# WangXuan95/NBLIC-Image-Compression

Measured on AMD Instinct MI355X. Metric: Mpixel/s encode (bit-exact) 4096x4096 gray -e1 lossless, higher is better.
Workload: dtype u8

## Files before the change

nblic-image-compression_amd/csrc/kernels_e1.h:

```cpp
#pragma once
#include <hip/hip_runtime.h>
#include <stdint.h>

namespace nblic {

constexpr uint32_t kMaxSegments = 1024;
constexpr uint32_t kTouchSegments = 256;
constexpr int kTotalsStride = 8, kWideTouchFlag = 4;
constexpr int kLongS2Met = 5, kLongS2Table = 6, kLongS2Serial = 7;
constexpr int kTotalsSlot = 16, kLongS3Split = 8, kLongS3Accepted = 9, kLongS3Missed = 10;
constexpr int kLongBlockMin = 128;

struct SegPlan { int nseg; uint32_t seg_len; };
SegPlan make_plan(uint32_t n_items, uint32_t max_segments = kMaxSegments);

constexpr size_t kStreamPad = 512;

struct E1Buffers {
    const uint8_t *img;
    uint32_t *rec1;
    uint16_t *s2in;
    uint32_t *pos2;
    uint16_t *s2out;
    uint16_t *pxs;
    uint16_t *s3in;
    uint32_t *pos3;
    uint16_t *s3out;
    uint8_t  *z;
    uint8_t  *cnt;
    uint32_t *ev_off;
    uint32_t *table;
    uint32_t *scan_sums;
    uint32_t *totals;
    int      *ctx_state;
    int      *map_state;
    int      *cnt_state;
    uint32_t *events;
    uint16_t *tin;
    uint64_t *tpos;
    uint16_t *tout;
    uint32_t *blk_base;
    int      *blk_end;
    uint8_t  *blk_ok;
    int      *blk_cand;
    uint32_t *blk_item;
    int      *blk_tab;
    uint32_t *mblk_base;
    uint32_t *mblk_cnt;
    uint32_t *mend_cnt;
    uint64_t *mblk_perm;
    uint32_t *qhist;
    unsigned long long *dbg_out;
    uint32_t *win_base;
    uint32_t *win_recs;
    uint16_t *coded;
};

struct E1Job {
    E1Buffers b;
    int h, w;
    uint32_t n;
    SegPlan pp;
    uint32_t n_ev;
    SegPlan pe;
    int dbg;
    int near, k_step;
    uint64_t ktab;
    int long_min, long_block;
    int row0;
    uint64_t *pack_rows;
    int pack_lane;
};

constexpr int kE1Kernels = 31;
constexpr int kE1Marks = kE1Kernels + 1;
struct E1Timers { hipEvent_t ev[kE1Marks]; uint64_t mask = ~0ull; };
constexpr uint64_t kRooflineStages = (1ull << 1) | (1ull << 26);
static const char *const kE1StageNames[kE1Kernels] = {
    "k_init_state", "k_predict",
    "k_adr_count", "scan_reduce.adr", "scan_sums.adr", "scan_apply.adr", "k_adr_scatter",
    "k_plan_blocks", "k_bias_blocks", "k_bias_fixup",
    "k_map_count", "scan_reduce.map", "scan_sums.map", "scan_apply.map", "k_map_scatter",
    "k_mapper_chains",
// ... 24 lines not shown
```

nblic-image-compression_amd/csrc/kernels_e1.hip:

```cpp
#include <hip/hip_runtime.h>
#include "model.h"
#include "kernels_e1.h"
#include "lsq_f64.h"
#include "serial_engine.h"

namespace nblic {

#define NB_GLOBAL __attribute__((address_space(1)))
typedef uint32_t u32x2 __attribute__((ext_vector_type(2)));
typedef uint32_t u32x4 __attribute__((ext_vector_type(4)));
typedef int i32x2 __attribute__((ext_vector_type(2)));
template <class T>
__device__ __forceinline__ NB_GLOBAL T *gptr(T *p) {
    return (NB_GLOBAL T *)p;
}

__device__ __forceinline__ int lane_id() { return int(threadIdx.x & 63); }
__device__ __forceinline__ uint64_t lanes_below() { return (1ull << lane_id()) - 1ull; }

__device__ __forceinline__ uint32_t xcd_block() {
    const uint32_t b = blockIdx.x, per = gridDim.x >> 3;
    return (b & 7u) * per + (b >> 3);
}

// ... 783 lines not shown
__global__ void __launch_bounds__(64) k_map_check(const E1Job *__restrict__ jobs) {
    __shared__ int count[kMapSyms][64];
    const E1Job &J = jobs[blockIdx.y];
    const auto base = gptr(J.b.mblk_base); const auto s3in = gptr(J.b.s3in); const auto s3out = gptr(J.b.s3out);
    const auto perm = gptr(J.b.mblk_perm); const auto cnt = gptr(J.b.mblk_cnt);
    const int lane = int(threadIdx.x);
    const int key = int(blockIdx.x) * kMapLanes + (lane < kMapLanes ? lane : 0);
    const uint32_t first = base[key], nb = lane < kMapLanes ? base[key + 1] - first : 0u;
    if (nb == 0u) return;
    uint32_t c_start, c_end;
    map_chain_range(J, key, c_start, c_end);
    const uint32_t B = map_block_records(J);
    Perm20 rank_of{perm[size_t(first) * 4 + 2], perm[size_t(first) * 4 + 3]};
    uint32_t accepted = 0, missed = 0;
    for (uint32_t b = 1; b < nb; b++) {
        const size_t it = size_t(first + b);
        if (perm[it * 4] == rank_of.lo && perm[it * 4 + 1] == rank_of.hi) {
            accepted++;
            rank_of = Perm20{perm[it * 4 + 2], perm[it * 4 + 3]};
            continue;
        }
        missed++;
        Perm20 sym_at{0, 0};
        for (int s = 0; s < kMapSyms; s++) {
            const int r = perm_get(rank_of, s);
            perm_set(sym_at, r, s); count[r][lane] = int(cnt[it * kMapSyms + s]);
        }
        const uint32_t lo = c_start + b * B, hi = min(c_end, lo + B);
        for (uint32_t r = lo; r < hi; r += 8u) {
            uint32_t y[8];
#pragma unroll
            for (int k = 0; k < 8; k++) y[k] = s3in[min(r + uint32_t(k), hi - 1u)];
#pragma unroll
            for (int k = 0; k < 8; k++)
                if (r + uint32_t(k) < hi) s3out[r + uint32_t(k)] = uint16_t(mapper_step(rank_of, sym_at, count, lane, int(y[k])));
        }
    }
    const auto st = gptr(J.b.map_state) + size_t(key) * (3 * kMapSyms);
    for (int s = 0; s < kMapSyms; s++) {
        const int r = perm_get(rank_of, s);
        st[s] = r; st[kMapSyms + r] = s; st[2 * kMapSyms + r] = int(gptr(J.b.mend_cnt)[key * kMapSyms + s]);
    }
    if (accepted) atomicAdd(J.b.totals + kLongS3Accepted, accepted);
    if (missed) atomicAdd(J.b.totals + kLongS3Missed, missed);
}

template <bool GEN, class Step>
__device__ __forceinline__ int walk_job(const E1Job &J, int qu, int qv, int z, Step step) {
    return GEN ? walk_symbol_t(J.k_step, J.ktab, qu, qv, z, step) : walk_symbol(kMinKStep, qu, qv, z, step);
}

template <bool GEN>
__global__ void __launch_bounds__(256) k_count_bins(const E1Job *__restrict__ jobs) {
    const E1Job &J = jobs[blockIdx.y];
    const auto rec1 = gptr(J.b.rec1); const auto s3out = gptr(J.b.s3out);
    const auto pos3 = gptr(J.b.pos3); const auto z = gptr(J.b.z); const auto cnt = gptr(J.b.cnt);
    uint32_t t = xcd_block() * 256u + threadIdx.x;
    if (t >= J.n) return;
    Level L = s1_level(rec1[t]);
    uint32_t p = pos3[t];
    int zz = (p >> 31) ? int(p & 0xFF) : int(s3out[p]);
    z[t] = uint8_t(zz);
    int c = 0;
    walk_job<GEN>(J, L.qu, L.qv, zz, [&](int, int, int, int bin) { c++; return bin; });
    cnt[t] = uint8_t(c);
}

template <bool GEN>
__global__ void __launch_bounds__(256) k_emit_bins(const E1Job *__restrict__ jobs) {
    const E1Job &J = jobs[blockIdx.y];
    const auto rec1 = gptr(J.b.rec1); const auto z = gptr(J.b.z);
    const auto ev_off = gptr(J.b.ev_off); const auto events = gptr(J.b.events);
    uint32_t t = xcd_block() * 256u + threadIdx.x;
    if (t >= J.n) return;
    Level L = s1_level(rec1[t]);
    auto out = events + ev_off[t];
    walk_job<GEN>(J, L.qu, L.qv, int(z[t]), [&](int qu, int qv, int node, int bin) {
        *out++ = pack_event(qu, qv, node, L.qw, bin);
        return bin;
    });
}

struct Touch { bool valid; uint32_t key; uint32_t payload; int slot; };

__device__ __forceinline__ Touch touch_of(uint32_t e, int parity) {
    const int qu = ev_qu(e), qv = ev_qv(e), node = ev_node(e), qw = ev_qw(e), bin = ev_bin(e);
    const bool same = qu == qv;
    const bool mine = (qu & 1) == parity;
    Touch t;
    t.valid = mine || (!same && qw != 0);
    const int tree = mine ? qu : qv;
    const int w1 = mine ? kWeightOne - qw : qw;
    t.slot = mine ? 0 : 1;
    t.key = uint32_t(parity) * 2048u + uint32_t(tree >> 1) * 256u + uint32_t(node);
    t.payload = uint32_t(w1) | (same ? uint32_t(qw) << 6 | 1u << 13 : 0u) | (uint32_t(bin) << 12);
    return t;
}

__global__ void __launch_bounds__(256) k_touch_count(const E1Job *__restrict__ jobs) {
    __shared__ uint32_t lds[4][4096];
    const E1Job &J = jobs[blockIdx.y];
    const auto events = gptr(J.b.events); const auto table = gptr(J.b.table);
    const uint32_t n_ev = J.n_ev; const SegPlan plan = J.pe;
    int seg = int(xcd_block()) * 4 + int(threadIdx.x >> 6);
    if (seg >= plan.nseg) return;
    if (seg == 0 && lane_id() == 0) gptr(J.b.totals)[kWideTouchFlag] = (J.dbg & 256) ? 1u : 0u;
    uint32_t *hist = lds[threadIdx.x >> 6];
    lds_fill<4096>(hist, 0);
    uint32_t lo = uint32_t(seg) * plan.seg_len, hi = min(n_ev, lo + plan.seg_len);
    for (uint32_t base = lo; base < hi; base += 512) {
        uint32_t e[8];
#pragma unroll
        for (int k = 0; k < 8; k++) e[k] = events[min(base + 64u * uint32_t(k) + uint32_t(lane_id()), hi - 1)];
#pragma unroll
        for (int k = 0; k < 8; k++) {
            if (base + 64u * uint32_t(k) + uint32_t(lane_id()) < hi) {
                Touch a = touch_of(e[k], 0), b = touch_of(e[k], 1);
                if (a.valid) atomicAdd(&hist[a.key], 1u);
                if (b.valid) atomicAdd(&hist[b.key], 1u);
            }
        }
    }
    for (int k = lane_id(); k < 4096; k += 64) table[size_t(k) * plan.nseg + seg] = hist[k];
}

constexpr int kStageSlots = 64, kStageRing = 64;
constexpr uint32_t kNoTouch = 0xFFFFFFFFu;
constexpr int kPosBits = 28;
constexpr uint32_t kPosMask = (1u << kPosBits) - 1u;
// ... 277 lines not shown
            vb_1 = c1 - (o_ex + (hw & one));
            const int slot = 2 + (n_halv < kMaxHalv ? n_halv : kMaxHalv);
            write_lane3(slot, H * kTpl + hk + 1, vb_s, vb_1, r0, r1, r2);
            n_halv++;
        }
        r2 = write_lane<1>(n_halv, r2);
        if (lane < 8) {
            const auto rec = recs + size_t(rec_i) * 24 + lane * 3;
            rec[0] = uint32_t(r0); rec[1] = uint32_t(r1); rec[2] = uint32_t(r2);
        }
        const uint32_t whole = read_lane(incl, 63);
        base_s = vb_s + int(whole >> 16);
        base_1 = vb_1 + int(whole & 0xFFFFu);
        n_halv_all += unsigned(n_halv);
        rec_i++;
    };
    const uint32_t last_window = first_window + ((end - 1 - first_window) / kWin) * kWin;
    auto fetch = [&](uint32_t window) { return in_w[(min(window, last_window) >> 3) + lane]; };
    u32x4 b0 = fetch(first_window), b1 = fetch(first_window + kWin), b2 = fetch(first_window + 2 * kWin), b3 = fetch(first_window + 3 * kWin);
    for (uint32_t window = first_window; window < end; window += 4 * kWin) {
        process(b0, window);
        b0 = fetch(window + 4 * kWin);
        if (window + kWin < end) process(b1, window + kWin);
        b1 = fetch(window + 5 * kWin);
        if (window + 2 * kWin < end) process(b2, window + 2 * kWin);
        b2 = fetch(window + 6 * kWin);
        if (window + 3 * kWin < end) process(b3, window + 3 * kWin);
        b3 = fetch(window + 7 * kWin);
    }
    if (lane == 0) cnt_state[key] = i32x2{base_s - base_1, base_1};
    if ((dbg & 8) && lane == 0 && end - start > 100000u) {
        const auto d = gptr(J.b.dbg_out) + 256 + (key & 255) * 4;
        d[0] = __builtin_amdgcn_s_memtime() - t_begin; d[1] = end - start; d[2] = rec_i - gptr(J.b.win_base)[key]; d[3] = n_halv_all;
    }
}

__global__ void __launch_bounds__(256) k_counter_probs(const E1Job *__restrict__ jobs) {
    const E1Job &J = jobs[blockIdx.y];
    const uint32_t g = blockIdx.x * 4u + (threadIdx.x >> 6);
    if (g >= gptr(J.b.win_base)[4096]) return;
    const int lane = lane_id();
    const auto r = (NB_GLOBAL const u32x4 *)gptr(J.b.win_recs) + size_t(g) * 6;
    const u32x4 r0 = r[0], r1 = r[1], r2 = r[2], r3 = r[3], r4 = r[4], r5 = r[5];
    const uint32_t window = r0.x, start = r0.y, end = r0.z;
    const int n_halv = min(int(r1.y), kMaxHalv + 1);
    const int from[kMaxHalv + 1] = {int(r1.z), int(r2.y), int(r3.x), int(r3.w), int(r4.z), int(r5.y)};
    const int hs[kMaxHalv + 1] = {int(r1.w), int(r2.z), int(r3.y), int(r4.x), int(r4.w), int(r5.z)};
    const int h1[kMaxHalv + 1] = {int(r2.x), int(r2.w), int(r3.z), int(r4.y), int(r5.x), int(r5.w)};
    const auto tin_g = gptr(J.b.tin); const auto tout = gptr(J.b.tout);
    const uint32_t first = window + uint32_t(lane) * kTpl;
    const u32x4 w = ((NB_GLOBAL const u32x4 *)tin_g)[first >> 3];
    uint32_t pay[kTpl]; int tin[kTpl], oin[kTpl], lane_t, lane_o;
    window_prefix(w, window, start, end, lane, pay, tin, oin, lane_t, lane_o);
    uint32_t p[kTpl];
#pragma unroll
    for (int k = 0; k < kTpl; k++) {
        const int j = lane * kTpl + k;
        int vs = int(r0.w), v1 = int(r1.x);
#pragma unroll
        for (int h = 0; h <= kMaxHalv; h++) if (h < n_halv && j >= from[h]) { vs = hs[h]; v1 = h1[h]; }
        const int t_ex = k ? tin[k - 1] : lane_t, o_ex = k ? oin[k - 1] : lane_o;
        p[k] = prob_one(v1 + o_ex, vs + t_ex);
    }
    if (first >= start && first + kTpl <= end) {
        ((NB_GLOBAL u32x4 *)tout)[first >> 3] = u32x4{p[0] | (p[1] << 16), p[2] | (p[3] << 16), p[4] | (p[5] << 16), p[6] | (p[7] << 16)};
    } else {
#pragma unroll
        for (int k = 0; k < kTpl; k++) if (first + k >= start && first + k < end) tout[first + k] = uint16_t(p[k]);
    }
}

__device__ __forceinline__ uint32_t mixed_code(const E1Job &J, uint32_t r, bool wide) {
    if (r >= J.n_ev) return 0u;
    const auto tout = gptr(J.b.tout);
    const auto pos0 = (NB_GLOBAL const uint32_t *)gptr(J.b.tpos);
    const auto pos1 = pos0 + ((size_t(J.n_ev) + 63) & ~size_t(63));
    uint32_t p0 = pos0[r], p1 = pos1[r];
    int qw, bin; bool odd;
    if (wide) {
        const uint32_t e = gptr(J.b.events)[r];
        qw = ev_qw(e); bin = ev_bin(e); odd = (ev_qu(e) & 1) != 0;
    } else {
        qw = int((p0 >> kPosBits) | (((p1 >> kPosBits) & 3u) << 4)); bin = int((p1 >> (kPosBits + 2)) & 1u); odd = (p1 >> 31) != 0u;
        p0 &= kPosMask; p1 &= kPosMask;
        if (p0 == kPosMask) p0 = kNoTouch;
        if (p1 == kPosMask) p1 = kNoTouch;
    }
    const uint32_t at_u = odd ? p1 : p0, other = odd ? p0 : p1, at_v = other == kNoTouch ? at_u : other;
    const int pu = tout[at_u], pv = tout[at_v];
    return uint32_t(mix_prob(pu, pv, qw)) | (uint32_t(bin) << 12);
}

__global__ void __launch_bounds__(256) k_mix(const E1Job *__restrict__ jobs) {
    const E1Job &J = jobs[blockIdx.y];
    const uint32_t r = xcd_block() * 256u + threadIdx.x;
    if ((r & ~63u) >= J.n_ev) return;
    const uint32_t code = mixed_code(J, r, gptr(J.b.totals)[kWideTouchFlag] != 0u);
    if (!J.pack_rows) {
        if (r < J.n_ev) gptr(J.b.coded)[r] = pack_coded(int(code & 0xFFFu), int(code >> 12));
        return;
    }
    const int lane = int(threadIdx.x) & 63;
    const int j = lane < kPackWords ? lane : kPackWords - 1;
    const uint32_t c0 = uint32_t(__builtin_amdgcn_ds_bpermute((4 * j + 0) << 2, int(code)));
    const uint32_t c1 = uint32_t(__builtin_amdgcn_ds_bpermute((4 * j + 1) << 2, int(code)));
    const uint32_t c2 = uint32_t(__builtin_amdgcn_ds_bpermute((4 * j + 2) << 2, int(code)));
    const uint32_t c3 = uint32_t(__builtin_amdgcn_ds_bpermute((4 * j + 3) << 2, int(code)));
    const uint32_t top_prob = uint32_t(__builtin_amdgcn_ds_bpermute((52 + (j < 12 ? j : 0)) << 2, int(code))) & 0xFFFu;
    const uint64_t ones = __ballot((code >> 12) != 0u);
    const uint64_t top = j < 12 ? uint64_t(top_prob) : ((ones >> 52) & 0xFFFull);
    const uint64_t word = uint64_t(c0) | (uint64_t(c1) << 13) | (uint64_t(c2) << 26) | (uint64_t(c3) << 39) | (top << 52);
    if (lane < kPackWords) ((NB_GLOBAL uint64_t *)gptr(J.b.tin))[size_t(r >> 6) * kPackWords + size_t(lane)] = word;
}

__global__ void __launch_bounds__(256) k_pack_rows(const E1Job *__restrict__ jobs, int n_jobs) {
// ... 17 lines not shown
    constexpr int kTile = 64;
    __shared__ int tile[kTile * 60];
    const IndexRecordTask T = tasks[blockIdx.x];
    const E1Job &J = jobs[T.job];
    const int t = int(threadIdx.x);
    const auto rec = gptr(out) + T.out;
    const auto words = (NB_GLOBAL uint32_t *)rec;
    constexpr int kHeadWords = int(sizeof(SerialState) / 4), kBiasWord = int(offsetof(SerialState, bias) / 4);
    if (t < kHeadWords) words[t] = t == kBiasWord ? uint32_t(lsq::kBiasInit) : 0u;
    const auto tab = words + kHeadWords;
    const auto ctx_state = gptr(J.b.ctx_state);
    for (int k = t; k < kContexts; k += 256) tab[k] = uint32_t(ctx_state[k]);
    const auto cnt_state = (NB_GLOBAL const i32x2 *)gptr(J.b.cnt_state);
    for (int key = t; key < 4096; key += 256) {
        const i32x2 c = cnt_state[key];
        const int tree = ((key >> 8) & 7) * 2 + (key >> 11), node = key & 255;
        tab[kContexts + tree * kTreeNodes + node] = uint32_t(c.x) | (uint32_t(c.y) << 16);
    }
    const auto map_state = gptr(J.b.map_state);
    const auto rank = rec + sizeof(SerialState) + size_t(kRecRank) * 4, sym = rec + sizeof(SerialState) + size_t(kRecSym) * 4;
    for (int m0 = 0; m0 < 512; m0 += kTile) {
        for (int k = t; k < kTile * 60; k += 256) tile[k] = map_state[m0 * 60 + k];
        __syncthreads();
        for (int k = t; k < kTile * kMapSyms; k += 256) {
            const int m = k / kMapSyms, q = k - m * kMapSyms;
            rank[m0 * kMapSyms + k] = uint8_t(tile[m * 60 + q]);
            sym[m0 * kMapSyms + k] = uint8_t(tile[m * 60 + 20 + q]);
            tab[kRecCount + m0 * kMapSyms + k] = uint32_t(tile[m * 60 + 40 + q]);
        }
        __syncthreads();
    }
    const int w = J.w, r = J.row0 + J.h, n = r < 2 ? r : 2;
    const auto rows = rec + kDecodeStateBytes;
    const auto img = gptr(J.b.img);
    const ptrdiff_t zeros = ptrdiff_t(2 - n) * w, from = ptrdiff_t(J.h - n) * w;
    for (ptrdiff_t k = t; k < 2 * ptrdiff_t(w); k += 256) rows[k] = k < zeros ? uint8_t(0) : img[from + (k - zeros)];
}

__global__ void k_init_state(const E1Job *__restrict__ jobs) {
    const E1Job &J = jobs[blockIdx.y];
    const auto ctx_state = gptr(J.b.ctx_state); const auto map_state = gptr(J.b.map_state); const auto cnt_state = (NB_GLOBAL i32x2 *)gptr(J.b.cnt_state);
    int g = int(blockIdx.x) * 256 + int(threadIdx.x);
    if (g < 3072) { ctx_state[g] = 0; gptr(J.b.qhist)[g] = 0; }
    if (g < 4096) cnt_state[g] = i32x2{kWeightOne, kWeightOne};
    if (g < 512)
        for (int k = 0; k < kMapSyms; k++) {
            map_state[g * 60 + k] = k; map_state[g * 60 + 20 + k] = k; map_state[g * 60 + 40 + k] = 2 * (kMapSyms - 1 - k);
        }
}

constexpr int kScanThreads = 256, kScanPerThread = 16, kScanTile = kScanThreads * kScanPerThread;

template <int WHICH> struct ScanSel;
template <> struct ScanSel<0> { typedef uint32_t T; static __device__ auto in(const E1Job &J) { return gptr(J.b.table); }  static __device__ auto out(const E1Job &J) { return gptr(J.b.table); }  static __device__ uint32_t n(const E1Job &J) { return uint32_t(kContexts) * J.pp.nseg; } };
template <> struct ScanSel<1> { typedef uint32_t T; static __device__ auto in(const E1Job &J) { return gptr(J.b.table); }  static __device__ auto out(const E1Job &J) { return gptr(J.b.table); }  static __device__ uint32_t n(const E1Job &J) { return 512u * J.pp.nseg; } };
template <> struct ScanSel<2> { typedef uint8_t  T; static __device__ auto in(const E1Job &J) { return gptr(J.b.cnt); }    static __device__ auto out(const E1Job &J) { return gptr(J.b.ev_off); } static __device__ uint32_t n(const E1Job &J) { return J.n; } };
template <> struct ScanSel<4> { typedef uint32_t T; static __device__ auto in(const E1Job &J) { return gptr(J.b.table); }  static __device__ auto out(const E1Job &J) { return gptr(J.b.table); }  static __device__ uint32_t n(const E1Job &J) { return 3072u * J.pp.nseg; } };
template <> struct ScanSel<3> { typedef uint32_t T; static __device__ auto in(const E1Job &J) { return gptr(J.b.table); }  static __device__ auto out(const E1Job &J) { return gptr(J.b.table); }  static __device__ uint32_t n(const E1Job &J) { return 4096u * J.pe.nseg; } };

template <int WHICH>
__global__ void __launch_bounds__(kScanThreads) k_scan_reduce(const E1Job *__restrict__ jobs) {
    __shared__ uint32_t part[kScanThreads / 64];
    const E1Job &J = jobs[blockIdx.y];
    const auto in = ScanSel<WHICH>::in(J);
    const uint32_t n = ScanSel<WHICH>::n(J);
    uint32_t base = blockIdx.x * uint32_t(kScanTile) + threadIdx.x * kScanPerThread, s = 0;
    if (blockIdx.x * uint32_t(kScanTile) >= n) return;
    for (int k = 0; k < kScanPerThread; k++) if (base + k < n) s += uint32_t(in[base + k]);
    s = wave_scan_incl(s);
    if (lane_id() == 63) part[threadIdx.x >> 6] = s;
    __syncthreads();
    if (threadIdx.x == 0) gptr(J.b.scan_sums)[blockIdx.x] = part[0] + part[1] + part[2] + part[3];
}

template <int WHICH>
__global__ void __launch_bounds__(1024) k_scan_sums(const E1Job *__restrict__ jobs) {
    __shared__ uint32_t part[16];
    __shared__ uint32_t carry;
    const E1Job &J = jobs[blockIdx.y];
    const auto sums = gptr(J.b.scan_sums);
    const uint32_t nblocks = (ScanSel<WHICH>::n(J) + kScanTile - 1) / kScanTile;
    if (threadIdx.x == 0) carry = 0;
    __syncthreads();
    for (uint32_t base = 0; base < nblocks; base += 1024) {
        uint32_t i = base + threadIdx.x;
        uint32_t v = i < nblocks ? sums[i] : 0u;
        uint32_t incl = wave_scan_incl(v);
        if (lane_id() == 63) part[threadIdx.x >> 6] = incl;
        __syncthreads();
        uint32_t pre = carry;
        for (int wv = 0; wv < int(threadIdx.x >> 6); wv++) pre += part[wv];
        if (i < nblocks) sums[i] = pre + incl - v;
        __syncthreads();
        if (threadIdx.x == 1023) carry = pre + incl;
        __syncthreads();
    }
    if (threadIdx.x == 0) {
        gptr(J.b.totals)[WHICH & 3] = carry;
        if (WHICH == 3 && carry >= kPosMask) gptr(J.b.totals)[kWideTouchFlag] = 1u;
    }
}

template <int WHICH>
__global__ void __launch_bounds__(kScanThreads) k_scan_apply(const E1Job *__restrict__ jobs) {
    __shared__ uint32_t part[kScanThreads / 64];
    const E1Job &J = jobs[blockIdx.y];
    const auto in = ScanSel<WHICH>::in(J);
    const auto out = ScanSel<WHICH>::out(J);
    const uint32_t n = ScanSel<WHICH>::n(J);
    if (blockIdx.x * uint32_t(kScanTile) >= n) return;
    uint32_t base = blockIdx.x * uint32_t(kScanTile) + threadIdx.x * kScanPerThread;
    uint32_t v[kScanPerThread], s = 0;
    for (int k = 0; k < kScanPerThread; k++) { v[k] = base + k < n ? uint32_t(in[base + k]) : 0u; s += v[k]; }
    uint32_t incl = wave_scan_incl(s);
    if (lane_id() == 63) part[threadIdx.x >> 6] = incl;
    __syncthreads();
    uint32_t pre = gptr(J.b.scan_sums)[blockIdx.x] + incl - s;
    for (int wv = 0; wv < int(threadIdx.x >> 6); wv++) pre += part[wv];
    for (int k = 0; k < kScanPerThread; k++) { if (base + k < n) out[base + k] = pre; pre += v[k]; }
}

__global__ void __launch_bounds__(256) k_q_predict(const E1Job *__restrict__ jobs) {
    const E1Job &J = jobs[blockIdx.z];
    const int w = J.w;
    int j = int(blockIdx.x) * 256 + int(threadIdx.x);
    int i = int(blockIdx.y);
    if (i >= J.h || j >= w) return;
    const auto img = gptr(J.b.img);
    auto pix = [&](int r, int c) { return int(img[size_t(r) * size_t(w) + size_t(c)]); };
    Taps n = sample_taps_q(pix, w, i, j);
    int px0 = predict_q(n);
    int err_prev = 0;
    if (j > 0) err_prev = pix(i, j - 1) - predict_q(sample_taps_q(pix, w, i, j - 1));
    int qd = level_q(n, err_prev);
    gptr(J.b.rec1)[size_t(i) * size_t(w) + size_t(j)] = uint32_t(px0) | (uint32_t(context_address_q(n, qd, px0)) << 8);
}

__global__ void __launch_bounds__(256) k_q_predict_band(const E1Job *__restrict__ jobs) {
    const E1Job &J = jobs[blockIdx.z];
    const int w = J.w, row0 = J.row0;
    int j = int(blockIdx.x) * 256 + int(threadIdx.x);
    int i = int(blockIdx.y);
    if (i >= J.h || j >= w) return;
    const auto img = gptr(J.b.img);
    auto pix = [&](int r, int c) { return int(img[(ptrdiff_t(r) - ptrdiff_t(row0)) * ptrdiff_t(w) + ptrdiff_t(c)]); };
    Taps n = sample_taps_q(pix, w, row0 + i, j);
    int px0 = predict_q(n);
    int err_prev = 0;
    if (j > 0) err_prev = pix(row0 + i, j - 1) - predict_q(sample_taps_q(pix, w, row0 + i, j - 1));
    int qd = level_q(n, err_prev);
    gptr(J.b.rec1)[size_t(i) * size_t(w) + size_t(j)] = uint32_t(px0) | (uint32_t(context_address_q(n, qd, px0)) << 8);
// ... 71 lines not shown

template <int WHICH>
static void scan_exclusive(const E1Job *jobs, int n_jobs, uint32_t max_items, hipStream_t s, Marker &mark) {
    unsigned nb = cdiv(max_items, kScanTile);
    if (nb == 0) nb = 1;
    mark(); hipLaunchKernelGGL(k_scan_reduce<WHICH>, dim3(nb, n_jobs), dim3(kScanThreads), 0, s, jobs);
    mark(); hipLaunchKernelGGL(k_scan_sums<WHICH>, dim3(1, n_jobs), dim3(1024), 0, s, jobs);
    mark(); hipLaunchKernelGGL(k_scan_apply<WHICH>, dim3(nb, n_jobs), dim3(kScanThreads), 0, s, jobs);
}

SegPlan make_plan(uint32_t n_items, uint32_t max_segments) {
    SegPlan p;
    uint32_t want = (n_items + max_segments - 1) / max_segments;
    if (want < 1024) want = 1024;
    p.seg_len = (want + 63u) & ~63u;
    p.nseg = int((n_items + p.seg_len - 1) / p.seg_len);
    if (p.nseg < 1) p.nseg = 1;
    return p;
}

static void launch_mapper_chains(const E1Job *d_jobs, const E1Job *h_jobs, int n_jobs, uint32_t max_n, hipStream_t s) {
    hipLaunchKernelGGL(k_mapper_chains, dim3(512 / kMapLanes, n_jobs), dim3(64), 0, s, d_jobs);
    if (h_jobs[0].long_min < 0) return;
    const unsigned B = unsigned(h_jobs[0].long_block > kLongBlockMin ? h_jobs[0].long_block : kLongBlockMin);
    const unsigned most = max_n / unsigned(h_jobs[0].long_min > 1 ? h_jobs[0].long_min : 1) + 1u;
    const unsigned max_blocks = max_n / B + (most < 512u ? most : 512u);
    hipLaunchKernelGGL(k_map_plan, dim3(1, n_jobs), dim3(512), 0, s, d_jobs);
    hipLaunchKernelGGL(k_map_hist, dim3(max_blocks, n_jobs), dim3(64), 0, s, d_jobs);
    hipLaunchKernelGGL(k_map_prefix, dim3(512, n_jobs), dim3(64), 0, s, d_jobs);
    hipLaunchKernelGGL(k_map_blocks, dim3(cdiv(max_blocks, kMapLanes), n_jobs), dim3(64), 0, s, d_jobs);
    hipLaunchKernelGGL(k_map_check, dim3(512 / kMapLanes, n_jobs), dim3(64), 0, s, d_jobs);
}

static void front_behind_s1(const E1Job *d_jobs, const E1Job *h_jobs, int n_jobs, int max_nseg, uint32_t max_n, hipStream_t s, Marker &mark, hipEvent_t model_done) {
    const bool long_chains = h_jobs[0].long_min >= 0;
    const dim3 seg_grid(pad8(cdiv(max_nseg, 4)), n_jobs), px_grid(pad8(cdiv(max_n, 256)), n_jobs);
    mark(); hipLaunchKernelGGL(k_adr_count<NbModel>, seg_grid, dim3(256), 0, s, d_jobs);
    scan_exclusive<0>(d_jobs, n_jobs, uint32_t(kContexts) * max_nseg, s, mark);
    mark(); hipLaunchKernelGGL(k_adr_scatter<NbModel>, seg_grid, dim3(256), 0, s, d_jobs);
    mark(); hipLaunchKernelGGL(k_plan_blocks<NbModel>, dim3(1, n_jobs), dim3(1024), 0, s, d_jobs);
    const unsigned max_blocks = max_n / kBiasBlock + unsigned(kContexts);
    mark(); hipLaunchKernelGGL(k_bias_blocks<NbModel>, dim3(cdiv(max_blocks, 64), n_jobs), dim3(64), 0, s, d_jobs);
    mark();
    const unsigned max_tabs = max_n / kBiasBlock + 1u;
    if (long_chains) hipLaunchKernelGGL(k_bias_tabulate<NbModel>, dim3(max_tabs, n_jobs), dim3(kBiasCands), 0, s, d_jobs);
    hipLaunchKernelGGL(k_bias_fixup<NbModel>, dim3(kContexts / 64, n_jobs), dim3(64), 0, s, d_jobs);
    if (long_chains) hipLaunchKernelGGL(k_bias_replay<NbModel>, dim3(cdiv(max_tabs, 64), n_jobs), dim3(64), 0, s, d_jobs);
    if (model_done) hipEventRecord(model_done, s);
    mark(); hipLaunchKernelGGL(k_map_count, seg_grid, dim3(256), 0, s, d_jobs);
    scan_exclusive<1>(d_jobs, n_jobs, 512u * max_nseg, s, mark);
    mark(); hipLaunchKernelGGL(k_map_scatter<false>, seg_grid, dim3(256), 0, s, d_jobs);
    mark(); launch_mapper_chains(d_jobs, h_jobs, n_jobs, max_n, s);
    mark(); hipLaunchKernelGGL(k_count_bins<false>, px_grid, dim3(256), 0, s, d_jobs);
    scan_exclusive<2>(d_jobs, n_jobs, max_n, s, mark);
    mark();
}

template <bool BAND>
static void launch_front(const E1Job *d_jobs, const E1Job *h_jobs, int n_jobs, hipStream_t s, E1Timers *tm, hipEvent_t model_done) {
    int max_w = 0, max_h = 0, max_nseg = 0; uint32_t max_n = 0;
    for (int k = 0; k < n_jobs; k++) {
        max_w = h_jobs[k].w > max_w ? h_jobs[k].w : max_w; max_h = h_jobs[k].h > max_h ? h_jobs[k].h : max_h;
        max_n = h_jobs[k].n > max_n ? h_jobs[k].n : max_n; max_nseg = h_jobs[k].pp.nseg > max_nseg ? h_jobs[k].pp.nseg : max_nseg;
    }
    Marker mark{tm, s, 0};
    if (!BAND) { mark(); hipLaunchKernelGGL(k_init_state, dim3(16, n_jobs), dim3(256), 0, s, d_jobs); }
    mark();
    if (BAND) {
        int top_rows = 0;
        for (int k = 0; k < n_jobs; k++) {
            const int t = 2 - h_jobs[k].row0 < h_jobs[k].h ? 2 - h_jobs[k].row0 : h_jobs[k].h;
            top_rows = t > top_rows ? t : top_rows;
        }
        if (max_h > 0 && max_w >= 20) hipLaunchKernelGGL(k_predict_rows<true>, dim3(cdiv((max_w - 12) / 8, 256), max_h, n_jobs), dim3(256), 0, s, d_jobs);
        if (top_rows > 0) hipLaunchKernelGGL(k_predict_border<true>, dim3(cdiv(max_w, 64), top_rows, n_jobs), dim3(64), 0, s, d_jobs, 1);
        hipLaunchKernelGGL(k_predict_border<true>, dim3(1, max_h, n_jobs), dim3(64), 0, s, d_jobs, 0);
    } else {
        if (max_h > 2 && max_w >= 20) hipLaunchKernelGGL(k_predict_rows<false>, dim3(cdiv((max_w - 12) / 8, 256), max_h - 2, n_jobs), dim3(256), 0, s, d_jobs);
        hipLaunchKernelGGL(k_predict_border<false>, dim3(cdiv(max_w, 64), max_h < 2 ? max_h : 2, n_jobs), dim3(64), 0, s, d_jobs, 1);
        if (max_h > 2) hipLaunchKernelGGL(k_predict_border<false>, dim3(1, max_h - 2, n_jobs), dim3(64), 0, s, d_jobs, 0);
    }
    front_behind_s1(d_jobs, h_jobs, n_jobs, max_nseg, max_n, s, mark, BAND ? model_done : nullptr);
}

void e1_launch_front(const E1Job *d_jobs, const E1Job *h_jobs, int n_jobs, hipStream_t s, E1Timers *tm) {
    launch_front<false>(d_jobs, h_jobs, n_jobs, s, tm, nullptr);
}

void e1_launch_front_band(const E1Job *d_jobs, const E1Job *h_jobs, int n_jobs, hipStream_t s, hipEvent_t model_done) {
    launch_front<true>(d_jobs, h_jobs, n_jobs, s, nullptr, model_done);
}

void e1_launch_model_stages(const E1Job *d_jobs, const E1Job *h_jobs, int n_jobs, hipStream_t s) {
    int max_nseg = 0; uint32_t max_n = 0;
    for (int k = 0; k < n_jobs; k++) {
        max_n = h_jobs[k].n > max_n ? h_jobs[k].n : max_n; max_nseg = h_jobs[k].pp.nseg > max_nseg ? h_jobs[k].pp.nseg : max_nseg;
    }
    Marker mark{nullptr, s, 0};
    front_behind_s1(d_jobs, h_jobs, n_jobs, max_nseg, max_n, s, mark, nullptr);
}

void e1_launch_front_pre(const E1Job *d_jobs, const E1Job *h_jobs, int n_jobs, hipStream_t s) {
    int max_nseg = 0; uint32_t max_n = 0;
    for (int k = 0; k < n_jobs; k++) {
        max_n = h_jobs[k].n > max_n ? h_jobs[k].n : max_n; max_nseg = h_jobs[k].pp.nseg > max_nseg ? h_jobs[k].pp.nseg : max_nseg;
    }
    const dim3 seg_grid(pad8(cdiv(max_nseg, 4)), n_jobs), px_grid(pad8(cdiv(max_n, 256)), n_jobs);
    Marker mark{nullptr, s, 0};
    hipLaunchKernelGGL(k_map_count_pre, seg_grid, dim3(256), 0, s, d_jobs);
    scan_exclusive<1>(d_jobs, n_jobs, 512u * max_nseg, s, mark);
    hipLaunchKernelGGL(k_map_scatter<true>, seg_grid, dim3(256), 0, s, d_jobs);
    launch_mapper_chains(d_jobs, h_jobs, n_jobs, max_n, s);
    hipLaunchKernelGGL(k_count_bins<true>, px_grid, dim3(256), 0, s, d_jobs);
    scan_exclusive<2>(d_jobs, n_jobs, max_n, s, mark);
}

void e1_launch_init(const E1Job *d_jobs, int n_jobs, hipStream_t s) {
    hipLaunchKernelGGL(k_init_state, dim3(16, n_jobs), dim3(256), 0, s, d_jobs);
}

void e1_launch_index_records(const E1Job *d_jobs, const IndexRecordTask *d_tasks, int n_tasks, uint8_t *d_out, hipStream_t s) {
    if (n_tasks > 0) hipLaunchKernelGGL(k_index_records, dim3(unsigned(n_tasks)), dim3(256), 0, s, d_jobs, d_tasks, d_out);
}

static void back_behind_emit(const E1Job *d_jobs, const E1Job *h_jobs, int n_jobs, int max_nseg, uint32_t max_ev, hipStream_t s, Marker &mark) {
    const dim3 seg_grid(pad8(cdiv(max_nseg, 4)), n_jobs);
    mark(); hipLaunchKernelGGL(k_touch_count, seg_grid, dim3(256), 0, s, d_jobs);
    scan_exclusive<3>(d_jobs, n_jobs, 4096u * max_nseg, s, mark);
    mark();
    if (h_jobs[0].dbg & 8) hipLaunchKernelGGL(k_touch_scatter<true>, dim3(seg_grid.x, seg_grid.y, 2), dim3(256), 0, s, d_jobs);
    else hipLaunchKernelGGL(k_touch_scatter<false>, dim3(seg_grid.x, seg_grid.y, 2), dim3(256), 0, s, d_jobs);
    mark(); hipLaunchKernelGGL(k_plan_windows, dim3(1, n_jobs), dim3(1024), 0, s, d_jobs);
    mark(); hipLaunchKernelGGL(k_counter_epochs, dim3(4096, n_jobs), dim3(64), 0, s, d_jobs);
    const unsigned max_windows = unsigned(2ull * max_ev / kWin) + 4096u;
    mark(); hipLaunchKernelGGL(k_counter_probs, dim3(cdiv(max_windows, 4), n_jobs), dim3(256), 0, s, d_jobs);
    mark(); hipLaunchKernelGGL(k_mix, dim3(pad8(cdiv(max_ev, 256) ? cdiv(max_ev, 256) : 1), n_jobs), dim3(256), 0, s, d_jobs);
    uint32_t pack_ev = 0;
    for (int k = 0; k < n_jobs; k++) if (h_jobs[k].pack_rows && h_jobs[k].n_ev > pack_ev) pack_ev = h_jobs[k].n_ev;
    if (pack_ev) hipLaunchKernelGGL(k_pack_rows, dim3(pad8(cdiv(cdiv(pack_ev, 64) * unsigned(kPackWords * kPackLanes), 256)), cdiv(unsigned(n_jobs), unsigned(kPackLanes))), dim3(256), 0, s, d_jobs, n_jobs);
    mark();
}

void e1_launch_back(const E1Job *d_jobs, const E1Job *h_jobs, int n_jobs, hipStream_t s, E1Timers *tm, bool general) {
    int max_nseg = 0; uint32_t max_n = 0, max_ev = 0;
    for (int k = 0; k < n_jobs; k++) {
        max_n = h_jobs[k].n > max_n ? h_jobs[k].n : max_n; max_ev = h_jobs[k].n_ev > max_ev ? h_jobs[k].n_ev : max_ev;
        max_nseg = h_jobs[k].pe.nseg > max_nseg ? h_jobs[k].pe.nseg : max_nseg;
    }
    Marker mark{tm, s, 21};
    mark();
    if (general) hipLaunchKernelGGL(k_emit_bins<true>, dim3(pad8(cdiv(max_n, 256)), n_jobs), dim3(256), 0, s, d_jobs);
    else hipLaunchKernelGGL(k_emit_bins<false>, dim3(pad8(cdiv(max_n, 256)), n_jobs), dim3(256), 0, s, d_jobs);
    back_behind_emit(d_jobs, h_jobs, n_jobs, max_nseg, max_ev, s, mark);
}

void e1_launch_back_stages(const E1Job *d_jobs, const E1Job *h_jobs, int n_jobs, hipStream_t s) {
    int max_nseg = 0; uint32_t max_ev = 0;
    for (int k = 0; k < n_jobs; k++) {
        max_ev = h_jobs[k].n_ev > max_ev ? h_jobs[k].n_ev : max_ev; max_nseg = h_jobs[k].pe.nseg > max_nseg ? h_jobs[k].pe.nseg : max_nseg;
    }
    Marker mark{nullptr, s, 22};
    back_behind_emit(d_jobs, h_jobs, n_jobs, max_nseg, max_ev, s, mark);
}

static void q_behind_predict(const E1Job *d_jobs, int n_jobs, int max_nseg, uint32_t max_n, bool long_chains, hipStream_t s) {
    const dim3 seg_grid(pad8(cdiv(max_nseg, 4)), n_jobs);
    Marker mark{nullptr, s, 0};
// ... 51 lines not shown
```

nblic-image-compression_amd/csrc/pipeline.hip:

```cpp
#include <hip/hip_runtime.h>

#include <algorithm>
#include <atomic>
#include <chrono>
#include <condition_variable>
#include <cstdio>
#include <cstdlib>
#include <cstring>
#include <deque>
#include <functional>
#include <memory>
#include <mutex>
#include <thread>
#include <type_traits>
#include <vector>

#include <pthread.h>
#include <sched.h>
#include <fcntl.h>
#include <unistd.h>

#include "../../include/nblic_amd.h"
#include "device_coder.h"
#include "hip_owned.h"
// ... 279 lines not shown
    c->fcv.notify_all();
}

static uint8_t *begin_stream_out(const ReadyImage &im, size_t *room) {
    const size_t cap = std::min(im.caps[im.job], size_t(1) << 46);
    *room = cap >= size_t(kHeaderBytes) ? cap - kHeaderBytes : 0;
    if (cap >= size_t(kHeaderBytes)) write_header(im.outs[im.job], im.h, im.w, im.near, im.k_step, im.effort);
    return im.outs[im.job] + kHeaderBytes;
}

static bool group_init(Group &g, int id, int n_slots, nblic_amd_ctx *c) {
    g.id = id; g.ctx = c;
    g.slots.resize(size_t(n_slots));
    HIP_OK(g.stream.create(hipStreamNonBlocking));
    HIP_OK(g.done.create(hipEventDisableTiming | hipEventBlockingSync));
    if (c->engine.available()) HIP_OK(g.released.create(hipEventDisableTiming | hipEventReleaseToSystem));
    for (int k = 0; k < kE1Marks; k++) { HIP_OK(g.tm_ev[k].create(hipEventDefault)); g.tm.ev[k] = g.tm_ev[k]; }
    HIP_OK(g.h_jobs.alloc(size_t(n_slots))); HIP_OK(g.d_jobs.alloc(size_t(n_slots)));
    HIP_OK(g.h_sjobs.alloc(size_t(n_slots))); HIP_OK(g.d_sjobs.alloc(size_t(n_slots)));
    HIP_OK(g.h_totals.alloc(size_t(n_slots) * kTotalsSlot)); HIP_OK(g.d_totals.alloc(size_t(n_slots) * kTotalsSlot));
    for (int k = 0; k < n_slots; k++) {
        Slot &s = g.slots[size_t(k)];
        DevPool &m = s.mem;
        HIP_OK(m.renew(s.b.table, size_t(4096) * kMaxSegments)); HIP_OK(m.renew(s.b.scan_sums, (size_t(1) << 20) / sizeof(uint32_t)));
        s.b.totals = g.d_totals + size_t(k) * kTotalsSlot;
        HIP_OK(m.renew(s.b.ctx_state, 4096));
        HIP_OK(m.renew(s.b.qhist, 12 * 256)); HIP_OK(m.renew(s.b.map_state, 512 * 60)); HIP_OK(m.renew(s.b.cnt_state, 4096 * 2));
        HIP_OK(m.renew(s.b.win_base, 4097 + 4096)); HIP_OK(m.renew(s.b.blk_base, 4097)); HIP_OK(m.renew(s.b.mblk_base, 513)); HIP_OK(m.renew(s.b.mend_cnt, 512 * 20)); HIP_OK(m.renew(s.b.dbg_out, 4096));
        HIP_OK(hipMemset(s.b.dbg_out, 0, 4096 * sizeof(unsigned long long)));
        uint8_t *state = nullptr;
        HIP_OK(m.renew(state, kModelStateBytes));
        s.d_state = reinterpret_cast<SerialState *>(state);
    }
    return true;
}

static bool ensure_events(Slot &s, size_t n_ev) {
    if (n_ev <= s.ev_cap) return true;
    const size_t cap = n_ev + n_ev / 8 + 1024;
    DevPool &m = s.mem;
    s.ev_cap = 0;
    HIP_OK(m.renew(s.b.events, cap)); HIP_OK(m.renew(s.b.tin, 2 * cap + kStreamPad)); HIP_OK(m.renew(s.b.tpos, cap + 64));
    HIP_OK(m.renew(s.b.tout, 2 * cap + kStreamPad)); HIP_OK(m.renew(s.b.win_recs, (2 * cap / 512 + 4096 + 8) * 24));
    s.ev_cap = cap;
    return true;
}

static bool ensure_pixels(Slot &s, size_t n, bool with_events = true) {
    if (n > s.px_cap) {
        DevPool &m = s.mem;
        s.px_cap = 0;
        HIP_OK(m.renew(s.b.rec1, n)); HIP_OK(m.renew(s.b.s2in, n + kStreamPad)); HIP_OK(m.renew(s.b.pos2, n)); HIP_OK(m.renew(s.b.s2out, n + kStreamPad));
        HIP_OK(m.renew(s.b.pxs, n)); HIP_OK(m.renew(s.b.s3in, n + kStreamPad)); HIP_OK(m.renew(s.b.pos3, n)); HIP_OK(m.renew(s.b.s3out, n + kStreamPad));
        HIP_OK(m.renew(s.b.z, n)); HIP_OK(m.renew(s.b.cnt, n)); HIP_OK(m.renew(s.b.ev_off, n));
        HIP_OK(m.renew(s.b.blk_end, n / 4096 + 4096 + 64)); HIP_OK(m.renew(s.b.blk_ok, n / 4096 + 4096 + 64));
        HIP_OK(m.renew(s.b.blk_cand, 2 * (n / 4096 + 4096 + 64))); HIP_OK(m.renew(s.b.blk_item, n / 4096 + 64)); HIP_OK(m.renew(s.b.blk_tab, 128 * (n / 4096 + 64)));
        HIP_OK(m.renew(s.b.mblk_cnt, 20 * (n / kLongBlockMin + 512))); HIP_OK(m.renew(s.b.mblk_perm, 4 * (n / kLongBlockMin + 512)));
        s.px_cap = n;
    }
    return with_events ? ensure_events(s, 5 * n) : true;
}

static void e1_job_back(E1Job &J, const E1Buffers &b, uint32_t n_ev, uint64_t *pack_rows = nullptr, int pack_lane = 0) {
    J.b = b; J.n_ev = n_ev; J.pe = make_plan(n_ev, kTouchSegments);
    J.pack_rows = pack_rows; J.pack_lane = pack_lane;
}

constexpr int kLongMinDefault = 65536, kLongBlockDefault = 4096;
struct LongChains { int min_records, block_records; };
static LongChains long_chains_of(const nblic_amd_ctx *c) {
    if (c->long_min < 0) return LongChains{-1, 0};
    return LongChains{c->long_min ? c->long_min : kLongMinDefault, std::max(c->long_block ? c->long_block : kLongBlockDefault, kLongBlockMin)};
}
static void count_long_chains(nblic_amd_ctx *c, const uint32_t *totals) {
    std::lock_guard<std::mutex> l(c->stat_m);
    c->long_counts[0] += totals[kLongS2Met]; c->long_counts[1] += totals[kLongS2Table]; c->long_counts[2] += totals[kLongS2Serial];
    c->long_counts[3] += totals[kLongS3Split]; c->long_counts[4] += totals[kLongS3Accepted]; c->long_counts[5] += totals[kLongS3Missed];
}

static E1Job e1_job_front(const E1Buffers &b, int rows, int w, int near, int dbg, LongChains lc) {
    E1Job J{};
    J.h = rows; J.w = w; J.n = uint32_t(size_t(rows) * size_t(w)); J.pp = make_plan(J.n); J.dbg = dbg;
    J.long_min = lc.min_records; J.long_block = lc.block_records;
    J.near = near; J.k_step = k_step_for_near(near); J.ktab = level_shift_table(J.k_step);
    e1_job_back(J, b, 0);
    return J;
}

static E1Job band_job_front(const nblic_amd_ctx *c, E1Buffers b, const uint8_t *plane, int row0, int rows, int w, int near) {
    b.img = plane + size_t(row0) * size_t(w);
    E1Job J = e1_job_front(b, rows, w, near, 0, long_chains_of(c));
    J.row0 = row0;
    return J;
}

static SerialJob model_job(const uint8_t *img, uint8_t *recon, const E1Buffers &b, double *stats, SerialState *state, int h, int w,
                           int near, int effort, int rows, int out_row0, unsigned long long *redo) {
    SerialJob Q{};
    Q.img = img; Q.recon = recon; Q.rec1 = b.rec1; Q.pxs = b.pxs; Q.stats = stats; Q.state = state;
    Q.h = h; Q.w = w; Q.near = near; Q.k_step = k_step_for_near(near); Q.effort = effort;
    Q.rows = rows; Q.out_row0 = out_row0; Q.redo = redo;
    return Q;
}

enum : uint8_t { kSrcRefused = 0, kSrcInPlace = 1, kSrcCollect = 2 };
struct CollectFrom {
    const nblic_amd_src *srcs; uint32_t format; float scale, bias;
// ... 4680 lines not shown
```

Before: 5456.

## Fuse bin-count scan into count/emit kernels via per-tile totals

k_count_bins now reduces each 256-pixel tile's bin counts with a wave DPP scan and writes one total per tile. The exclusive scan then runs only over these tile totals instead of every per-pixel count. k_emit_bins rebuilds each pixel's event offset from the scanned tile base plus an in-block scan, and writes ev_off itself. Separately, the counter-probability kernel hoists the halving-segment lookup out of the per-element loop, using one current/next boundary per lane. This trades a full-size scan pass for a small amount of extra in-block scan work, at the cost of added shared-memory syncs in the two kernels.

```diff
diff --git a/nblic-image-compression_amd/csrc/kernels_e1.h b/nblic-image-compression_amd/csrc/kernels_e1.h
--- a/nblic-image-compression_amd/csrc/kernels_e1.h
+++ b/nblic-image-compression_amd/csrc/kernels_e1.h
@@ -29,6 +29,7 @@
     uint8_t  *z;
     uint8_t  *cnt;
     uint32_t *ev_off;
+    uint32_t *bin_tiles;
     uint32_t *table;
     uint32_t *scan_sums;
     uint32_t *totals;
diff --git a/nblic-image-compression_amd/csrc/kernels_e1.hip b/nblic-image-compression_amd/csrc/kernels_e1.hip
--- a/nblic-image-compression_amd/csrc/kernels_e1.hip
+++ b/nblic-image-compression_amd/csrc/kernels_e1.hip
@@ -859,29 +859,46 @@
 
 template <bool GEN>
 __global__ void __launch_bounds__(256) k_count_bins(const E1Job *__restrict__ jobs) {
+    __shared__ uint32_t part[4];
     const E1Job &J = jobs[blockIdx.y];
     const auto rec1 = gptr(J.b.rec1); const auto s3out = gptr(J.b.s3out);
     const auto pos3 = gptr(J.b.pos3); const auto z = gptr(J.b.z); const auto cnt = gptr(J.b.cnt);
-    uint32_t t = xcd_block() * 256u + threadIdx.x;
-    if (t >= J.n) return;
-    Level L = s1_level(rec1[t]);
-    uint32_t p = pos3[t];
-    int zz = (p >> 31) ? int(p & 0xFF) : int(s3out[p]);
-    z[t] = uint8_t(zz);
+    const uint32_t tile = xcd_block(), t = tile * 256u + threadIdx.x;
+    if (tile * 256u >= J.n) return;
     int c = 0;
-    walk_job<GEN>(J, L.qu, L.qv, zz, [&](int, int, int, int bin) { c++; return bin; });
-    cnt[t] = uint8_t(c);
+    if (t < J.n) {
+        Level L = s1_level(rec1[t]);
+        uint32_t p = pos3[t];
+        int zz = (p >> 31) ? int(p & 0xFF) : int(s3out[p]);
+        z[t] = uint8_t(zz);
+        walk_job<GEN>(J, L.qu, L.qv, zz, [&](int, int, int, int bin) { c++; return bin; });
+        cnt[t] = uint8_t(c);
+    }
+    const uint32_t incl = wave_scan_incl_dpp(uint32_t(c));
+    if (lane_id() == 63) part[threadIdx.x >> 6] = incl;
+    __syncthreads();
+    if (threadIdx.x == 0) gptr(J.b.bin_tiles)[tile] = part[0] + part[1] + part[2] + part[3];
 }
 
 template <bool GEN>
 __global__ void __launch_bounds__(256) k_emit_bins(const E1Job *__restrict__ jobs) {
+    __shared__ uint32_t part[4];
     const E1Job &J = jobs[blockIdx.y];
     const auto rec1 = gptr(J.b.rec1); const auto z = gptr(J.b.z);
     const auto ev_off = gptr(J.b.ev_off); const auto events = gptr(J.b.events);
-    uint32_t t = xcd_block() * 256u + threadIdx.x;
+    const uint32_t tile = xcd_block(), t = tile * 256u + threadIdx.x;
+    if (tile * 256u >= J.n) return;
+    const uint32_t c = t < J.n ? uint32_t(gptr(J.b.cnt)[t]) : 0u;
+    const uint32_t incl = wave_scan_incl_dpp(c);
+    const int wave = int(threadIdx.x >> 6);
+    if (lane_id() == 63) part[wave] = incl;
+    __syncthreads();
+    uint32_t off = gptr(J.b.bin_tiles)[tile] + incl - c;
+    off += (wave > 0 ? part[0] : 0u) + (wave > 1 ? part[1] : 0u) + (wave > 2 ? part[2] : 0u);
     if (t >= J.n) return;
+    ev_off[t] = off;
     Level L = s1_level(rec1[t]);
-    auto out = events + ev_off[t];
+    auto out = events + off;
     walk_job<GEN>(J, L.qu, L.qv, int(z[t]), [&](int qu, int qv, int node, int bin) {
         *out++ = pack_event(qu, qv, node, L.qw, bin);
         return bin;
@@ -1265,15 +1282,19 @@
     const u32x4 w = ((NB_GLOBAL const u32x4 *)tin_g)[first >> 3];
     uint32_t pay[kTpl]; int tin[kTpl], oin[kTpl], lane_t, lane_o;
     window_prefix(w, window, start, end, lane, pay, tin, oin, lane_t, lane_o);
+    const int j0 = lane * kTpl;
+    int vs = int(r0.w), v1 = int(r1.x);
+    int next = int(kWin), ns = vs, n1 = v1;
+#pragma unroll
+    for (int h = 0; h <= kMaxHalv; h++) if (h < n_halv && from[h] <= j0) { vs = hs[h]; v1 = h1[h]; }
+#pragma unroll
+    for (int h = kMaxHalv; h >= 0; h--) if (h < n_halv && from[h] > j0) { next = from[h]; ns = hs[h]; n1 = h1[h]; }
     uint32_t p[kTpl];
 #pragma unroll
     for (int k = 0; k < kTpl; k++) {
-        const int j = lane * kTpl + k;
-        int vs = int(r0.w), v1 = int(r1.x);
-#pragma unroll
-        for (int h = 0; h <= kMaxHalv; h++) if (h < n_halv && j >= from[h]) { vs = hs[h]; v1 = h1[h]; }
+        const bool behind = j0 + k >= next;
         const int t_ex = k ? tin[k - 1] : lane_t, o_ex = k ? oin[k - 1] : lane_o;
-        p[k] = prob_one(v1 + o_ex, vs + t_ex);
+        p[k] = prob_one((behind ? n1 : v1) + o_ex, (behind ? ns : vs) + t_ex);
     }
     if (first >= start && first + kTpl <= end) {
         ((NB_GLOBAL u32x4 *)tout)[first >> 3] = u32x4{p[0] | (p[1] << 16), p[2] | (p[3] << 16), p[4] | (p[5] << 16), p[6] | (p[7] << 16)};
@@ -1397,11 +1418,11 @@
 constexpr int kScanThreads = 256, kScanPerThread = 16, kScanTile = kScanThreads * kScanPerThread;
 
 template <int WHICH> struct ScanSel;
-template <> struct ScanSel<0> { typedef uint32_t T; static __device__ auto in(const E1Job &J) { return gptr(J.b.table); }  static __device__ auto out(const E1Job &J) { return gptr(J.b.table); }  static __device__ uint32_t n(const E1Job &J) { return uint32_t(kContexts) * J.pp.nseg; } };
-template <> struct ScanSel<1> { typedef uint32_t T; static __device__ auto in(const E1Job &J) { return gptr(J.b.table); }  static __device__ auto out(const E1Job &J) { return gptr(J.b.table); }  static __device__ uint32_t n(const E1Job &J) { return 512u * J.pp.nseg; } };
-template <> struct ScanSel<2> { typedef uint8_t  T; static __device__ auto in(const E1Job &J) { return gptr(J.b.cnt); }    static __device__ auto out(const E1Job &J) { return gptr(J.b.ev_off); } static __device__ uint32_t n(const E1Job &J) { return J.n; } };
-template <> struct ScanSel<4> { typedef uint32_t T; static __device__ auto in(const E1Job &J) { return gptr(J.b.table); }  static __device__ auto out(const E1Job &J) { return gptr(J.b.table); }  static __device__ uint32_t n(const E1Job &J) { return 3072u * J.pp.nseg; } };
-template <> struct ScanSel<3> { typedef uint32_t T; static __device__ auto in(const E1Job &J) { return gptr(J.b.table); }  static __device__ auto out(const E1Job &J) { return gptr(J.b.table); }  static __device__ uint32_t n(const E1Job &J) { return 4096u * J.pe.nseg; } };
+template <> struct ScanSel<0> { static constexpr int kTotal = 0; static __device__ auto in(const E1Job &J) { return gptr(J.b.table); }  static __device__ auto out(const E1Job &J) { return gptr(J.b.table); }  static __device__ uint32_t n(const E1Job &J) { return uint32_t(kContexts) * J.pp.nseg; } };
+template <> struct ScanSel<1> { static constexpr int kTotal = 1; static __device__ auto in(const E1Job &J) { return gptr(J.b.table); }  static __device__ auto out(const E1Job &J) { return gptr(J.b.table); }  static __device__ uint32_t n(const E1Job &J) { return 512u * J.pp.nseg; } };
+template <> struct ScanSel<4> { static constexpr int kTotal = 0; static __device__ auto in(const E1Job &J) { return gptr(J.b.table); }  static __device__ auto out(const E1Job &J) { return gptr(J.b.table); }  static __device__ uint32_t n(const E1Job &J) { return 3072u * J.pp.nseg; } };
+template <> struct ScanSel<3> { static constexpr int kTotal = 3; static __device__ auto in(const E1Job &J) { return gptr(J.b.table); }  static __device__ auto out(const E1Job &J) { return gptr(J.b.table); }  static __device__ uint32_t n(const E1Job &J) { return 4096u * J.pe.nseg; } };
+template <> struct ScanSel<5> { static constexpr int kTotal = 2; static __device__ auto in(const E1Job &J) { return gptr(J.b.bin_tiles); } static __device__ auto out(const E1Job &J) { return gptr(J.b.bin_tiles); } static __device__ uint32_t n(const E1Job &J) { return J.n / 256u + uint32_t(J.n % 256u != 0u); } };
 
 template <int WHICH>
 __global__ void __launch_bounds__(kScanThreads) k_scan_reduce(const E1Job *__restrict__ jobs) {
@@ -1441,7 +1462,7 @@
         __syncthreads();
     }
     if (threadIdx.x == 0) {
-        gptr(J.b.totals)[WHICH & 3] = carry;
+        gptr(J.b.totals)[ScanSel<WHICH>::kTotal] = carry;
         if (WHICH == 3 && carry >= kPosMask) gptr(J.b.totals)[kWideTouchFlag] = 1u;
     }
 }
@@ -1619,7 +1640,7 @@
     mark(); hipLaunchKernelGGL(k_map_scatter<false>, seg_grid, dim3(256), 0, s, d_jobs);
     mark(); launch_mapper_chains(d_jobs, h_jobs, n_jobs, max_n, s);
     mark(); hipLaunchKernelGGL(k_count_bins<false>, px_grid, dim3(256), 0, s, d_jobs);
-    scan_exclusive<2>(d_jobs, n_jobs, max_n, s, mark);
+    scan_exclusive<5>(d_jobs, n_jobs, cdiv(max_n, 256), s, mark);
     mark();
 }
 
@@ -1679,7 +1700,7 @@
     hipLaunchKernelGGL(k_map_scatter<true>, seg_grid, dim3(256), 0, s, d_jobs);
     launch_mapper_chains(d_jobs, h_jobs, n_jobs, max_n, s);
     hipLaunchKernelGGL(k_count_bins<true>, px_grid, dim3(256), 0, s, d_jobs);
-    scan_exclusive<2>(d_jobs, n_jobs, max_n, s, mark);
+    scan_exclusive<5>(d_jobs, n_jobs, cdiv(max_n, 256), s, mark);
 }
 
 void e1_launch_init(const E1Job *d_jobs, int n_jobs, hipStream_t s) {
diff --git a/nblic-image-compression_amd/csrc/pipeline.hip b/nblic-image-compression_amd/csrc/pipeline.hip
--- a/nblic-image-compression_amd/csrc/pipeline.hip
+++ b/nblic-image-compression_amd/csrc/pipeline.hip
@@ -355,7 +355,7 @@
         s.px_cap = 0;
         HIP_OK(m.renew(s.b.rec1, n)); HIP_OK(m.renew(s.b.s2in, n + kStreamPad)); HIP_OK(m.renew(s.b.pos2, n)); HIP_OK(m.renew(s.b.s2out, n + kStreamPad));
         HIP_OK(m.renew(s.b.pxs, n)); HIP_OK(m.renew(s.b.s3in, n + kStreamPad)); HIP_OK(m.renew(s.b.pos3, n)); HIP_OK(m.renew(s.b.s3out, n + kStreamPad));
-        HIP_OK(m.renew(s.b.z, n)); HIP_OK(m.renew(s.b.cnt, n)); HIP_OK(m.renew(s.b.ev_off, n));
+        HIP_OK(m.renew(s.b.z, n)); HIP_OK(m.renew(s.b.cnt, n)); HIP_OK(m.renew(s.b.ev_off, n)); HIP_OK(m.renew(s.b.bin_tiles, n / 256 + 1));
         HIP_OK(m.renew(s.b.blk_end, n / 4096 + 4096 + 64)); HIP_OK(m.renew(s.b.blk_ok, n / 4096 + 4096 + 64));
         HIP_OK(m.renew(s.b.blk_cand, 2 * (n / 4096 + 4096 + 64))); HIP_OK(m.renew(s.b.blk_item, n / 4096 + 64)); HIP_OK(m.renew(s.b.blk_tab, 128 * (n / 4096 + 64)));
         HIP_OK(m.renew(s.b.mblk_cnt, 20 * (n / kLongBlockMin + 512))); HIP_OK(m.renew(s.b.mblk_perm, 4 * (n / kLongBlockMin + 512)));
```

Result: slower. 5341 (-2.1%).
